# jinli99/iShapEditing

Hardware: AMD Instinct MI355X
Metric: end-to-end drag-edit wall-clock (s) per shape (lower is better)
Workload: dtype f16; 1 GPU; C3 chair drag-edit: 3 handle->target pairs, 40 guided iterations (UNet fwd + drag gradient + UNet input-grad bwd + DDPM update) + 256^3 occupancy decode; unet=421M params, 1x96x128x128 latent, fp16 torso, r1=12, scale=1200

## Files before the change

ishapediting_amd/csrc/decode.hip:

```cpp
#include "decode.h"

#define LDH 136
#define LDB 36

__global__ void planes_prepare_kernel(const float* __restrict__ latent, const float* __restrict__ rng,
                                      const float* __restrict__ mid, float* __restrict__ planes, int S) {
  __shared__ float tile[32][33];
  const int p = blockIdx.z;
  const int pix0 = blockIdx.x * 32;
  const int tx = threadIdx.x & 31, ty = threadIdx.x >> 5;
  const int SS = S * S;
  for (int j = ty; j < 32; j += 8) {
    int c = p * 32 + j;
    float r = rng ? rng[c] : 1.f, m = mid ? mid[c] : 0.f;
    tile[j][tx] = latent[(long long)c * SS + pix0 + tx] * r + m;
  }
  __syncthreads();
  for (int j = ty; j < 32; j += 8)
    planes[((long long)p * SS + pix0 + j) * 32 + tx] = tile[tx][j];
}
int planes_prepare_launch(const float* latent, const float* rng, const float* mid, float* planes, int S, hipStream_t s) {
  ISHAP_REQUIRE(S >= 1 && ((long long)S * S) % 32 == 0, "planes_prepare: S * S must be a positive multiple of 32");
  hipLaunchKernelGGL(planes_prepare_kernel, dim3(S * S / 32, 1, 3), dim3(256), 0, s, latent, rng, mid, planes, S);
  ISHAP_CHECK_HIP(hipGetLastError());
  return 0;
}

__global__ __launch_bounds__(512) void triplane_decode_kernel(DecodeArgs a) {
  extern __shared__ __attribute__((aligned(16))) float lds[];
  half_t* sW1h = reinterpret_cast<half_t*>(lds);
  half_t* sW1l = sW1h + 128 * LDH;
  half_t* sW2h = sW1l + 128 * LDH;
  half_t* sW2l = sW2h + 128 * LDH;
  float* sBt = reinterpret_cast<float*>(sW2l + 128 * LDH);
  float* sb1 = sBt + 64 * LDB;
  float* sb2 = sb1 + 128;
  float* sw3 = sb2 + 128;
  const int tid = threadIdx.x;
  for (int i = tid; i < 128 * 128; i += 512) {
    const int r = i >> 7, p = i & 127;
    const int j = p & 7, hh = (p >> 3) & 1, st = (p >> 4) & 1, qb = p >> 5;
    const int k = 32 * qb + 16 * st + 8 * (j >> 2) + 4 * hh + (j & 3);
    const float w1 = a.W1[r * 128 + k], w2 = a.W2[r * 128 + k];
    const half_t h1 = (half_t)w1, h2 = (half_t)w2;
    sW1h[r * LDH + p] = h1; sW1l[r * LDH + p] = (half_t)(w1 - (float)h1);
    sW2h[r * LDH + p] = h2; sW2l[r * LDH + p] = (half_t)(w2 - (float)h2);
  }
  for (int i = tid; i < 64 * 32; i += 512) {
    int y = i >> 5, k = i & 31;
    sBt[y * LDB + k] = a.B[k * 64 + y];
  }
  if (tid < 128) { sb1[tid] = a.b1[tid]; sb2[tid] = a.b2[tid]; sw3[tid] = a.w3[tid]; }
  __syncthreads();

  const int lane = tid & 63;
  const int wave = tid >> 6;
  const int l31 = lane & 31, h = lane >> 5;
  const int S = a.S;
  const float b3 = a.b3[0];
  const long long ntiles = (a.npts + 31) / 32;
  const float two_pi = 6.2831855f;

  for (long long tile = (long long)blockIdx.x * 8 + wave; tile < ntiles; tile += (long long)gridDim.x * 8) {
    long long pt = tile * 32 + l31;
    const bool valid = pt < a.npts;
    if (!valid) pt = a.npts - 1;
    float cx, cy, cz;
    if (a.coords) {
      cx = a.coords[pt * 3 + 0]; cy = a.coords[pt * 3 + 1]; cz = a.coords[pt * 3 + 2];
    } else {
      const int res = a.res;
      int k = (int)(pt % res);
      long long ij = pt / res;
      int j = (int)(ij % res), i = (int)(ij / res);
      cx = a.lin[i]; cy = a.lin[j]; cz = a.lin[k];
    }
    f32x4 f[4];
#pragma unroll
    for (int g = 0; g < 4; ++g) f[g] = (f32x4){0.f, 0.f, 0.f, 0.f};
#pragma unroll
    for (int p = 0; p < 3; ++p) {
      const float u = (p == 1) ? cy : cx;
      const float v = (p == 0) ? cy : cz;
      const float ix = ((u + 1.f) / 2.f) * (float)(S - 1);
      const float iy = ((v + 1.f) / 2.f) * (float)(S - 1);
      const float fx = floorf(ix), fy = floorf(iy);
      const int x0 = (int)fx, y0 = (int)fy;
      const float wx1 = ix - fx, wx0 = (fx + 1.f) - ix;
      const float wy1 = iy - fy, wy0 = (fy + 1.f) - iy;
      const float* pl = a.planes + (long long)p * S * S * 32;
      f32x4 acc[4];
#pragma unroll
      for (int g = 0; g < 4; ++g) acc[g] = (f32x4){0.f, 0.f, 0.f, 0.f};
#pragma unroll
      for (int q = 0; q < 4; ++q) {
        const int xx = x0 + (q & 1), yy = y0 + (q >> 1);
        const float w = ((q & 1) ? wx1 : wx0) * ((q >> 1) ? wy1 : wy0);
        if (xx >= 0 && xx < S && yy >= 0 && yy < S) {
          const float* t = pl + ((long long)yy * S + xx) * 32 + 4 * h;
#pragma unroll
          for (int g = 0; g < 4; ++g) acc[g] += w * *reinterpret_cast<const f32x4*>(t + 8 * g);
        }
      }
#pragma unroll
      for (int g = 0; g < 4; ++g) f[g] += acc[g];
    }
    f32x16 d0[2];
#pragma unroll
    for (int q = 0; q < 2; ++q) {
#pragma unroll
      for (int r = 0; r < 16; ++r) d0[q][r] = 0.f;
#pragma unroll
      for (int g = 0; g < 4; ++g) {
        f32x4 av = *reinterpret_cast<const f32x4*>(sBt + (32 * q + l31) * LDB + 8 * g + 4 * h);
#pragma unroll
        for (int e = 0; e < 4; ++e) d0[q] = __builtin_amdgcn_mfma_f32_32x32x2f32(av[e], f[g][e], d0[q], 0, 0, 0);
      }
    }
    f32x16 x1[4];
#pragma unroll
    for (int q = 0; q < 2; ++q)
#pragma unroll
      for (int r = 0; r < 16; ++r) {
        const float ang = two_pi * d0[q][r];
        const float turns = ang * 0.15915494309189535f;
        const float fr = __builtin_amdgcn_fractf(turns);
        const float sv = __builtin_amdgcn_sinf(fr), cv = __builtin_amdgcn_cosf(fr);
        x1[q][r] = sv;
        x1[2 + q][r] = cv;
      }
    half8 xh[4][2], xl[4][2];
    auto split = [&](const f32x16 (&x)[4]) {
#pragma unroll
      for (int qb = 0; qb < 4; ++qb)
#pragma unroll
        for (int st = 0; st < 2; ++st)
#pragma unroll
          for (int j = 0; j < 8; ++j) {
            const float v = x[qb][8 * st + j];
            const half_t hi = (half_t)v;
            xh[qb][st][j] = hi;
            xl[qb][st][j] = (half_t)(v - (float)hi);
          }
    };
    auto layer = [&](const half_t* wh, const half_t* wl, int q) {
      f32x16 d;
#pragma unroll
      for (int r = 0; r < 16; ++r) d[r] = 0.f;
#pragma unroll
      for (int qb = 0; qb < 4; ++qb)
#pragma unroll
        for (int st = 0; st < 2; ++st) {
          const int off = (32 * q + l31) * LDH + ((qb * 2 + st) * 2 + h) * 8;
          const half8 ah = *reinterpret_cast<const half8*>(wh + off);
          const half8 al = *reinterpret_cast<const half8*>(wl + off);
          d = __builtin_amdgcn_mfma_f32_32x32x16_f16(ah, xh[qb][st], d, 0, 0, 0);
          d = __builtin_amdgcn_mfma_f32_32x32x16_f16(al, xh[qb][st], d, 0, 0, 0);
          d = __builtin_amdgcn_mfma_f32_32x32x16_f16(ah, xl[qb][st], d, 0, 0, 0);
          __builtin_amdgcn_sched_barrier(0);
        }
      return d;
    };
    split(x1);
    f32x16 x2[4];
#pragma unroll
    for (int q = 0; q < 4; ++q) {
      x2[q] = layer(sW1h, sW1l, q);
#pragma unroll
      for (int r = 0; r < 16; ++r) x2[q][r] = fmaxf(x2[q][r] + sb1[32 * q + kmap(r, h)], 0.f);
    }
    split(x2);
    float partial = 0.f;
#pragma unroll
    for (int q = 0; q < 4; ++q) {
      const f32x16 d = layer(sW2h, sW2l, q);
#pragma unroll
      for (int r = 0; r < 16; ++r) {
        int nrn = 32 * q + kmap(r, h);
        partial += sw3[nrn] * fmaxf(d[r] + sb2[nrn], 0.f);
      }
    }
    partial += __shfl_xor(partial, 32);
    if (h == 0 && valid) a.out[pt] = partial + b3;
  }
}

int triplane_decode_launch(const DecodeArgs& a, hipStream_t s) {
  ISHAP_REQUIRE(a.npts > 0, "triplane decode: no points");
  ISHAP_REQUIRE(a.S >= 1, "triplane decode: plane size");
  ISHAP_REQUIRE(a.coords != nullptr || (a.lin != nullptr && a.res > 0), "either coords or a grid axis");
  const size_t smem = (size_t)4 * 128 * LDH * sizeof(half_t) + (size_t)(64 * LDB + 3 * 128) * sizeof(float);
  ISHAP_TRY(ishap_set_max_lds((const void*)triplane_decode_kernel, (int)smem));
  long long ntiles = (a.npts + 31) / 32;
  int blocks = (int)std::min<long long>((ntiles + 7) / 8, 256);
  hipLaunchKernelGGL(triplane_decode_kernel, dim3(blocks), dim3(512), smem, s, a);
  ISHAP_CHECK_HIP(hipGetLastError());
  return 0;
}
```

Measured before the change: 0.1617 s/shape.

## Software-pipeline triplane gathers for next tile behind current tile's MLP MFMAs

Restructures the triplane decode loop so the bilinear plane taps of the next tile are issued and reduced in pieces between the current tile's Fourier and MLP MFMA phases. Global-memory gather latency is meant to hide behind matrix work, and sched_barrier calls fix the interleaving. Also adds branchless clamped tap loads, 32-bit index division for grid coordinates, and precomputed per-lane LDS pointers. The cost is much higher register pressure from holding prefetched taps, which could reduce occupancy or cause spills. It only touches the 256^3 decode stage.

```diff
diff --git a/ishapediting_amd/csrc/decode.hip b/ishapediting_amd/csrc/decode.hip
--- a/ishapediting_amd/csrc/decode.hip
+++ b/ishapediting_amd/csrc/decode.hip
@@ -1,4 +1,5 @@
 #include "decode.h"
+#include <type_traits>
 
 #define LDH 136
 #define LDB 36
@@ -24,6 +25,80 @@
   hipLaunchKernelGGL(planes_prepare_kernel, dim3(S * S / 32, 1, 3), dim3(256), 0, s, latent, rng, mid, planes, S);
   ISHAP_CHECK_HIP(hipGetLastError());
   return 0;
+}
+
+struct PlaneTaps {
+  f32x4 t[4][4];
+  float w[4];
+  bool ok[4];
+};
+
+__device__ __forceinline__ void tile_coords(const DecodeArgs& a, long long tile, int l31, float& cx, float& cy, float& cz) {
+  long long pt = tile * 32 + l31;
+  if (pt >= a.npts) pt = a.npts - 1;
+  if (a.coords) {
+    cx = a.coords[pt * 3 + 0]; cy = a.coords[pt * 3 + 1]; cz = a.coords[pt * 3 + 2];
+  } else {
+    const int res = a.res;
+    int i, j, k;
+    if (a.npts <= 0x7fffffffLL) {
+      const unsigned up = (unsigned)pt, ur = (unsigned)res;
+      const unsigned ij = up / ur;
+      k = (int)(up - ij * ur);
+      i = (int)(ij / ur);
+      j = (int)(ij - (unsigned)i * ur);
+    } else {
+      k = (int)(pt % res);
+      const long long ij = pt / res;
+      j = (int)(ij % res); i = (int)(ij / res);
+    }
+    cx = a.lin[i]; cy = a.lin[j]; cz = a.lin[k];
+  }
+}
+
+__device__ __forceinline__ void taps_issue(const DecodeArgs& a, int p, int h, float cx, float cy, float cz, PlaneTaps& T) {
+#pragma clang fp contract(off)
+  const int S = a.S;
+  const float sm1 = (float)(S - 1);
+  const float u = (p == 1) ? cy : cx;
+  const float v = (p == 0) ? cy : cz;
+  const float mu = (u + 1.f) / 2.f, mv = (v + 1.f) / 2.f;
+  const float ix = mu * sm1, iy = mv * sm1;
+  const float fx = floorf(ix), fy = floorf(iy);
+  const int x0 = (int)fx, y0 = (int)fy;
+  const float wx1 = ix - fx, wx0 = __builtin_fmaf(-mu, sm1, fx + 1.f);
+  const float wy1 = iy - fy, wy0 = __builtin_fmaf(-mv, sm1, fy + 1.f);
+  const float* pl = a.planes + (long long)p * S * S * 32;
+#pragma unroll
+  for (int q = 0; q < 4; ++q) {
+    const int xx = x0 + (q & 1), yy = y0 + (q >> 1);
+    T.w[q] = ((q & 1) ? wx1 : wx0) * ((q >> 1) ? wy1 : wy0);
+    T.ok[q] = xx >= 0 && xx < S && yy >= 0 && yy < S;
+    const int xc = min(max(xx, 0), S - 1), yc = min(max(yy, 0), S - 1);
+    const float* t = pl + ((long long)yc * S + xc) * 32 + 4 * h;
+#pragma unroll
+    for (int g = 0; g < 4; ++g) T.t[q][g] = *reinterpret_cast<const f32x4*>(t + 8 * g);
+  }
+}
+
+__device__ __forceinline__ void taps_reduce(const PlaneTaps& T, f32x4 (&f)[4]) {
+#pragma clang fp contract(off)
+  f32x4 acc[4];
+#pragma unroll
+  for (int g = 0; g < 4; ++g) acc[g] = (f32x4){0.f, 0.f, 0.f, 0.f};
+#pragma unroll
+  for (int q = 0; q < 4; ++q)
+#pragma unroll
+    for (int g = 0; g < 4; ++g)
+#pragma unroll
+      for (int e = 0; e < 4; ++e) {
+        const float n = __builtin_fmaf(T.w[q], T.t[q][g][e], acc[g][e]);
+        acc[g][e] = T.ok[q] ? n : acc[g][e];
+      }
+#pragma unroll
+  for (int g = 0; g < 4; ++g) f[g] += acc[g];
+#pragma unroll
+  for (int g = 0; g < 4; ++g) asm volatile("" : "+v"(f[g]));
 }
 
 __global__ __launch_bounds__(512) void triplane_decode_kernel(DecodeArgs a) {
@@ -54,57 +129,43 @@
   __syncthreads();
 
   const int lane = tid & 63;
-  const int wave = tid >> 6;
+  const int wave = __builtin_amdgcn_readfirstlane(tid >> 6);
   const int l31 = lane & 31, h = lane >> 5;
-  const int S = a.S;
   const float b3 = a.b3[0];
   const long long ntiles = (a.npts + 31) / 32;
+  const long long stride = (long long)gridDim.x * 8;
   const float two_pi = 6.2831855f;
-
-  for (long long tile = (long long)blockIdx.x * 8 + wave; tile < ntiles; tile += (long long)gridDim.x * 8) {
-    long long pt = tile * 32 + l31;
-    const bool valid = pt < a.npts;
-    if (!valid) pt = a.npts - 1;
+  const int wlane = l31 * LDH + 8 * h;
+  const half_t *lW1h = sW1h + wlane, *lW1l = sW1l + wlane, *lW2h = sW2h + wlane, *lW2l = sW2l + wlane;
+  const float* lBt = sBt + l31 * LDB + 4 * h;
+  const float *lb1 = sb1 + 4 * h, *lb2 = sb2 + 4 * h, *lw3 = sw3 + 4 * h;
+
+  long long tile = (long long)blockIdx.x * 8 + wave;
+  if (tile >= ntiles) return;
+  f32x4 f[4];
+  float nx = 0.f, ny = 0.f, nz = 0.f;
+  {
+    PlaneTaps T;
     float cx, cy, cz;
-    if (a.coords) {
-      cx = a.coords[pt * 3 + 0]; cy = a.coords[pt * 3 + 1]; cz = a.coords[pt * 3 + 2];
-    } else {
-      const int res = a.res;
-      int k = (int)(pt % res);
-      long long ij = pt / res;
-      int j = (int)(ij % res), i = (int)(ij / res);
-      cx = a.lin[i]; cy = a.lin[j]; cz = a.lin[k];
-    }
-    f32x4 f[4];
+    tile_coords(a, tile, l31, cx, cy, cz);
+    bool more = tile + stride < ntiles;
+    if (more) tile_coords(a, tile + stride, l31, nx, ny, nz);
 #pragma unroll
     for (int g = 0; g < 4; ++g) f[g] = (f32x4){0.f, 0.f, 0.f, 0.f};
 #pragma unroll
     for (int p = 0; p < 3; ++p) {
-      const float u = (p == 1) ? cy : cx;
-      const float v = (p == 0) ? cy : cz;
-      const float ix = ((u + 1.f) / 2.f) * (float)(S - 1);
-      const float iy = ((v + 1.f) / 2.f) * (float)(S - 1);
-      const float fx = floorf(ix), fy = floorf(iy);
-      const int x0 = (int)fx, y0 = (int)fy;
-      const float wx1 = ix - fx, wx0 = (fx + 1.f) - ix;
-      const float wy1 = iy - fy, wy0 = (fy + 1.f) - iy;
-      const float* pl = a.planes + (long long)p * S * S * 32;
-      f32x4 acc[4];
-#pragma unroll
-      for (int g = 0; g < 4; ++g) acc[g] = (f32x4){0.f, 0.f, 0.f, 0.f};
-#pragma unroll
-      for (int q = 0; q < 4; ++q) {
-        const int xx = x0 + (q & 1), yy = y0 + (q >> 1);
-        const float w = ((q & 1) ? wx1 : wx0) * ((q >> 1) ? wy1 : wy0);
-        if (xx >= 0 && xx < S && yy >= 0 && yy < S) {
-          const float* t = pl + ((long long)yy * S + xx) * 32 + 4 * h;
-#pragma unroll
-          for (int g = 0; g < 4; ++g) acc[g] += w * *reinterpret_cast<const f32x4*>(t + 8 * g);
-        }
-      }
-#pragma unroll
-      for (int g = 0; g < 4; ++g) f[g] += acc[g];
-    }
+      taps_issue(a, p, h, cx, cy, cz, T);
+      taps_reduce(T, f);
+    }
+  }
+  auto one_tile = [&](auto prefetch) __attribute__((always_inline)) {
+    constexpr bool has_next = decltype(prefetch)::value;
+    const bool has_next2 = has_next && tile + 2 * stride < ntiles;
+    asm volatile("" ::: "memory");
+    PlaneTaps T0, T1, T2;
+    f32x4 fn[4];
+    if constexpr (has_next) taps_issue(a, 0, h, nx, ny, nz, T0);
+    __builtin_amdgcn_sched_barrier(0);
     f32x16 d0[2];
 #pragma unroll
     for (int q = 0; q < 2; ++q) {
@@ -112,7 +173,7 @@
       for (int r = 0; r < 16; ++r) d0[q][r] = 0.f;
 #pragma unroll
       for (int g = 0; g < 4; ++g) {
-        f32x4 av = *reinterpret_cast<const f32x4*>(sBt + (32 * q + l31) * LDB + 8 * g + 4 * h);
+        f32x4 av = *reinterpret_cast<const f32x4*>(lBt + 32 * q * LDB + 8 * g);
 #pragma unroll
         for (int e = 0; e < 4; ++e) d0[q] = __builtin_amdgcn_mfma_f32_32x32x2f32(av[e], f[g][e], d0[q], 0, 0, 0);
       }
@@ -151,7 +212,7 @@
       for (int qb = 0; qb < 4; ++qb)
 #pragma unroll
         for (int st = 0; st < 2; ++st) {
-          const int off = (32 * q + l31) * LDH + ((qb * 2 + st) * 2 + h) * 8;
+          const int off = 32 * q * LDH + (qb * 2 + st) * 16;
           const half8 ah = *reinterpret_cast<const half8*>(wh + off);
           const half8 al = *reinterpret_cast<const half8*>(wl + off);
           d = __builtin_amdgcn_mfma_f32_32x32x16_f16(ah, xh[qb][st], d, 0, 0, 0);
@@ -161,28 +222,56 @@
         }
       return d;
     };
+    __builtin_amdgcn_sched_barrier(0);
+    if constexpr (has_next) {
+#pragma unroll
+      for (int g = 0; g < 4; ++g) fn[g] = (f32x4){0.f, 0.f, 0.f, 0.f};
+      taps_reduce(T0, fn);
+    }
+    __builtin_amdgcn_sched_barrier(0);
     split(x1);
+    __builtin_amdgcn_sched_barrier(0);
+    if constexpr (has_next) taps_issue(a, 1, h, nx, ny, nz, T1);
+    __builtin_amdgcn_sched_barrier(0);
     f32x16 x2[4];
 #pragma unroll
     for (int q = 0; q < 4; ++q) {
-      x2[q] = layer(sW1h, sW1l, q);
-#pragma unroll
-      for (int r = 0; r < 16; ++r) x2[q][r] = fmaxf(x2[q][r] + sb1[32 * q + kmap(r, h)], 0.f);
+      x2[q] = layer(lW1h, lW1l, q);
+#pragma unroll
+      for (int r = 0; r < 16; ++r) x2[q][r] = fmaxf(x2[q][r] + lb1[32 * q + kmap(r, 0)], 0.f);
+      __builtin_amdgcn_sched_barrier(0);
+      if constexpr (has_next) { if (q == 1) taps_reduce(T1, fn); }
     }
     split(x2);
+    __builtin_amdgcn_sched_barrier(0);
+    float mx = 0.f, my = 0.f, mz = 0.f;
+    if constexpr (has_next) taps_issue(a, 2, h, nx, ny, nz, T2);
+    if (has_next2) tile_coords(a, tile + 2 * stride, l31, mx, my, mz);
+    __builtin_amdgcn_sched_barrier(0);
     float partial = 0.f;
 #pragma unroll
     for (int q = 0; q < 4; ++q) {
-      const f32x16 d = layer(sW2h, sW2l, q);
+      const f32x16 d = layer(lW2h, lW2l, q);
 #pragma unroll
       for (int r = 0; r < 16; ++r) {
-        int nrn = 32 * q + kmap(r, h);
-        partial += sw3[nrn] * fmaxf(d[r] + sb2[nrn], 0.f);
-      }
+        const int nrn = 32 * q + kmap(r, 0);
+        partial += lw3[nrn] * fmaxf(d[r] + lb2[nrn], 0.f);
+      }
+      __builtin_amdgcn_sched_barrier(0);
+      if constexpr (has_next) { if (q == 1) taps_reduce(T2, fn); }
     }
     partial += __shfl_xor(partial, 32);
-    if (h == 0 && valid) a.out[pt] = partial + b3;
-  }
+    const long long pt = tile * 32 + l31;
+    if (h == 0 && pt < a.npts) a.out[pt] = partial + b3;
+    if constexpr (has_next) {
+#pragma unroll
+      for (int g = 0; g < 4; ++g) f[g] = fn[g];
+      nx = mx; ny = my; nz = mz;
+      tile += stride;
+    }
+  };
+  while (tile + stride < ntiles) one_tile(std::true_type{});
+  one_tile(std::false_type{});
 }
 
 int triplane_decode_launch(const DecodeArgs& a, hipStream_t s) {
```

Result: no change. 0.1620 s/shape (+0.2%).
